# gregbugaj/marie-icr

Hardware: AMD Instinct MI355X
Metric: pages/sec (2550x3300, ~40 lines/page) (higher is better)
Workload: dtype f16; 1 GPU; BASELINE configs[2]: full detect->crop->recognize, 64 synthetic 2550x3300x3 u8 pages per GPU per step resident in HBM; DiT-base Mask R-CNN detector (resize to 1035x800, 1 pass, 8 pages per forward) + TrOCR-base recognizer on the generator's 40 ground-truth line boxes per page (fixed work), beam 3, 15+1 decoder steps; seeded random weights; f16 operands with fp32 accumulation is the 16-bit mode of ; crops_per_page=40

## Files before the change

include/marie_hip.h:

```cpp
#ifndef MARIE_HIP_H
#define MARIE_HIP_H

#include <stddef.h>
#include <stdint.h>

#ifdef __cplusplus
extern "C" {
#endif

#define MHIP_OK 0
#define MHIP_EINVAL (-22)
#define MHIP_ENOMEM (-12)
#define MHIP_EHIP (-5)
#define MHIP_ESTATE (-1)

#define MHIP_PREC_F16 0
#define MHIP_PREC_F32 1

typedef struct mhip_ctx mhip_ctx;
typedef struct mhip_crnn mhip_crnn;

int mhip_init(int device_id, mhip_ctx** out);
int mhip_destroy(mhip_ctx* ctx);
const char* mhip_last_error(mhip_ctx* ctx);
int mhip_set_stream(mhip_ctx* ctx, void* hip_stream);
int mhip_synchronize(mhip_ctx* ctx);
int mhip_device_info(mhip_ctx* ctx, char* arch, size_t arch_len, int* cu_count, size_t* hbm_bytes);
int mhip_memcpy_dev(mhip_ctx* ctx, void* dst_dev, const void* src_dev, size_t bytes);

typedef struct mhip_gate mhip_gate;
int mhip_gate_create(mhip_ctx* ctx, mhip_gate** out);
int mhip_gate_destroy(mhip_gate* g);
int mhip_gate_signal(mhip_gate* g, mhip_ctx* ctx);
long long mhip_gate_count(mhip_gate* g);
int mhip_gate_open(mhip_gate* g, int open);
int mhip_gate_wait(mhip_gate* g, mhip_ctx* ctx, long long seq, int timeout_ms);

int mhip_profile_enable(mhip_ctx* ctx, int enable);
int mhip_profile_reset(mhip_ctx* ctx);
int mhip_profile_read(mhip_ctx* ctx, int kernel_id, double* total_ms, int64_t* launches);
int mhip_profile_flops(mhip_ctx* ctx, int kernel_id, double* flops);
int mhip_kernel_count(void);
const char* mhip_kernel_name(int kernel_id);

typedef struct mhip_conv_desc {
  int32_t B, H, W, Cin;
  int32_t KH, KW, pad;
  int32_t N;
  int32_t pool, relu, out_f32;
  int32_t dil;
  int32_t Cin1;
  int32_t ldc;
  int32_t pad_cols_writable;
} mhip_conv_desc;
int mhip_conv2d_nhwc(mhip_ctx* ctx, int precision, const mhip_conv_desc* d, const void* in_dev,
                     const void* in2_dev, const void* w_dev, const float* scale_dev, const float* bias_dev,
                     void* out_dev);

typedef struct mhip_crop_desc {
  uint64_t src_offset;
  int32_t h, w, row_stride, channels;
} mhip_crop_desc;
int mhip_crop_batch(mhip_ctx* ctx, const uint8_t* base_dev, const mhip_crop_desc* descs_host, int n, int img_w,
                    uint8_t* out_dev);

int mhip_crnn_create(mhip_ctx* ctx, int precision, int num_class, mhip_crnn** out);
int mhip_crnn_destroy(mhip_crnn* m);

int mhip_crnn_set_tensor(mhip_crnn* m, const char* key, const float* data_host, const int64_t* shape, int ndim);
int mhip_crnn_finalize(mhip_crnn* m);
int mhip_crnn_alloc_arena(mhip_crnn* m);
int mhip_crnn_arena(mhip_crnn* m, void** arena_dev, size_t* bytes);

int mhip_crnn_seq_len(int w);

int mhip_crnn_forward(mhip_crnn* m, const uint8_t* crops_dev, int n, int w, float* logits_dev,
                      int32_t* argmax_dev, int32_t* tokens_dev, int32_t* lengths_dev, float* conf_dev);
int mhip_crnn_forward_host(mhip_crnn* m, const uint8_t* crops_host, int n, int w, float* logits_host,
                           int32_t* argmax_host, int32_t* tokens_host, int32_t* lengths_host,
                           float* conf_host);
int mhip_crnn_forward_crops(mhip_crnn* m, const uint8_t* base_dev, const mhip_crop_desc* descs_host, int n, int img_w,
                            float* logits_host, int32_t* argmax_host, int32_t* tokens_host, int32_t* lengths_host,
                            float* conf_host);
int mhip_crnn_forward_fragments_host(mhip_crnn* m, const uint8_t* packed_host, size_t packed_bytes,
                                     const mhip_crop_desc* descs_host, int n, int img_w, float* logits_host,
                                     int32_t* argmax_host, int32_t* tokens_host, int32_t* lengths_host,
                                     float* conf_host);
size_t mhip_crnn_workspace_bytes(mhip_crnn* m, int n, int w);
double mhip_crnn_kernel_flops(mhip_crnn* m, int kernel_id, int n, int w);

// ... 301 lines not shown
```

marie_icr_amd/_lib.py:

```python
from __future__ import annotations

import ctypes as C
import os
import weakref

import numpy as np

_HERE = os.path.dirname(os.path.abspath(__file__))
LIB_PATH = os.environ.get("MARIE_HIP_LIB") or os.path.join(_HERE, "libmarie_hip.so")

PREC_F16 = 0
PREC_F32 = 1

_vp, _i, _sz = C.c_void_p, C.c_int, C.c_size_t
_SIGNATURES = (
    ("mhip_init", _i, [_i, C.POINTER(_vp)]),
    ("mhip_destroy", _i, [_vp]),
    ("mhip_last_error", C.c_char_p, [_vp]),
    ("mhip_set_stream", _i, [_vp, _vp]),
    ("mhip_synchronize", _i, [_vp]),
    ("mhip_device_info", _i, [_vp, C.c_char_p, _sz, C.POINTER(_i), C.POINTER(_sz)]),
    ("mhip_memcpy_dev", _i, [_vp, _vp, _vp, _sz]),
    ("mhip_gate_create", _i, [_vp, C.POINTER(_vp)]),
    ("mhip_gate_destroy", _i, [_vp]),
    ("mhip_gate_signal", _i, [_vp, _vp]),
    ("mhip_gate_count", C.c_longlong, [_vp]),
    ("mhip_gate_open", _i, [_vp, _i]),
    ("mhip_gate_wait", _i, [_vp, _vp, C.c_longlong, _i]),
    ("mhip_profile_enable", _i, [_vp, _i]),
    ("mhip_profile_reset", _i, [_vp]),
    ("mhip_profile_read", _i, [_vp, _i, C.POINTER(C.c_double), C.POINTER(C.c_int64)]),
    ("mhip_profile_flops", _i, [_vp, _i, C.POINTER(C.c_double)]),
    ("mhip_kernel_count", _i, []),
    ("mhip_kernel_name", C.c_char_p, [_i]),
    ("mhip_conv2d_nhwc", _i, [_vp, _i, _vp, _vp, _vp, _vp, _vp, _vp, _vp]),
    ("mhip_icr_create", _i, [_vp, _i, _i, C.POINTER(_vp)]),
    ("mhip_icr_destroy", _i, [_vp]),
    ("mhip_icr_set_tensor", _i, [_vp, C.c_char_p, _vp, C.POINTER(C.c_int64), _i]),
    ("mhip_icr_finalize", _i, [_vp]),
    ("mhip_icr_alloc_arena", _i, [_vp]),
    ("mhip_icr_arena", _i, [_vp, C.POINTER(_vp), C.POINTER(_sz)]),
    ("mhip_icr_steps", _i, []),
    ("mhip_icr_forward", _i, [_vp, _vp, _i, _vp, _vp, _vp, _vp]),
    ("mhip_icr_forward_host", _i, [_vp, _vp, _i, _vp, _vp, _vp, _vp]),
    ("mhip_craft_create", _i, [_vp, _i, C.POINTER(_vp)]),
    ("mhip_craft_destroy", _i, [_vp]),
    ("mhip_craft_set_tensor", _i, [_vp, C.c_char_p, _vp, C.POINTER(C.c_int64), _i]),
    ("mhip_craft_finalize", _i, [_vp]),
    ("mhip_craft_alloc_arena", _i, [_vp]),
    ("mhip_craft_arena", _i, [_vp, C.POINTER(_vp), C.POINTER(_sz)]),
    ("mhip_craft_geometry", _i, [_i, _i, _i, C.c_double, C.POINTER(C.c_double), C.POINTER(_i), C.POINTER(_i),
                                 C.POINTER(_i), C.POINTER(_i)]),
    ("mhip_craft_workspace_bytes", _sz, [_vp, _i, _i, _i, C.c_double]),
    ("mhip_craft_kernel_flops", C.c_double, [_vp, _i, _i, _i, _i, C.c_double]),
    ("mhip_craft_forward", _i, [_vp, _vp, _i, _i, _i, C.c_double, _vp]),
    ("mhip_craft_detect", _i, [_vp, _vp, _i, _i, _i, C.c_double, C.c_float, C.c_float, C.c_float, _vp, _i,
                               C.POINTER(_i), _vp, C.POINTER(C.c_double)]),
    ("mhip_craft_detect_host", _i, [_vp, _vp, _i, _i, _i, C.c_double, C.c_float, C.c_float, C.c_float, _vp, _i,
                                    C.POINTER(_i), _vp, C.POINTER(C.c_double)]),
    ("mhip_craft_boxes_host", _i, [_vp, _vp, _i, _i, C.c_float, C.c_float, C.c_float, _vp, _i, C.POINTER(_i), _vp, _vp,
                                   _vp, _i, C.POINTER(_i)]),
    ("mhip_crop_batch", _i, [_vp, _vp, _vp, _i, _i, _vp]),
    ("mhip_pil_resize_rgb_host", _i, [_vp, _vp, _i, _i, _vp, _i, _i, _i]),
    ("mhip_vit_create", _i, [_vp, _i, _vp, C.POINTER(_vp)]),
    ("mhip_vit_destroy", _i, [_vp]),
    ("mhip_vit_set_tensor", _i, [_vp, C.c_char_p, _vp, C.POINTER(C.c_int64), _i]),
    ("mhip_vit_finalize", _i, [_vp]),
    ("mhip_vit_alloc_arena", _i, [_vp]),
# ... 80 lines not shown
    ("mhip_vq_kmeans_step_host", _i, [_vp, _vp, _i, _i, _vp, _vp, _i, _vp, _vp, _vp, C.POINTER(C.c_double)]),
    ("mhip_vq_heatmap_host", _i, [_vp, _vp, _i, _i, _i, _vp, _vp, _vp, _vp]),
    ("mhip_vq_peaks_host", _i, [_vp, _vp, _i, _i, _i, _vp, _i, _vp]),
    ("mhip_clip_cosine_host", _i, [_vp, _vp, _vp, _i, _i, _i, _vp]),
    ("mhip_max_page_size", _i, [_i, _i, _i, _i, C.c_double, C.POINTER(_i), C.POINTER(_i)]),
    ("mhip_resize_area_u8", _i, [_vp, _vp, _i, _i, _i, C.c_size_t, _vp, _i, _i]),
    ("mhip_resize_area_u8_host", _i, [_vp, _vp, _i, _i, _i, _vp, _i, _i]),
    ("mhip_resize_cubic_u8", _i, [_vp, _vp, _i, _i, _i, C.c_size_t, _vp, _i, _i]),
    ("mhip_resize_cubic_u8_host", _i, [_vp, _vp, _i, _i, _i, _vp, _i, _i]),
    ("mhip_merge_boxes", _i, [_vp, _i, _vp, C.POINTER(_i)]),
    ("mhip_line_merge", _i, [_vp, _i, _vp, C.POINTER(_i)]),
    ("mhip_find_line_numbers", _i, [_vp, _i, _vp, _i, _vp]),
    ("mhip_lines_from_bboxes", _i, [_vp, _i, _i, _i, _vp, _i, C.POINTER(_i)]),
    ("mhip_crnn_forward_crops", _i, [_vp, _vp, _vp, _i, _i, _vp, _vp, _vp, _vp, _vp]),
    ("mhip_crnn_forward_fragments_host", _i, [_vp, _vp, _sz, _vp, _i, _i, _vp, _vp, _vp, _vp, _vp]),
    ("mhip_crnn_create", _i, [_vp, _i, _i, C.POINTER(_vp)]),
    ("mhip_crnn_destroy", _i, [_vp]),
    ("mhip_crnn_set_tensor", _i, [_vp, C.c_char_p, _vp, C.POINTER(C.c_int64), _i]),
    ("mhip_crnn_finalize", _i, [_vp]),
    ("mhip_crnn_alloc_arena", _i, [_vp]),
    ("mhip_crnn_arena", _i, [_vp, C.POINTER(_vp), C.POINTER(_sz)]),
    ("mhip_crnn_seq_len", _i, [_i]),
    ("mhip_crnn_forward", _i, [_vp, _vp, _i, _i, _vp, _vp, _vp, _vp, _vp]),
    ("mhip_crnn_forward_host", _i, [_vp, _vp, _i, _i, _vp, _vp, _vp, _vp, _vp]),
    ("mhip_crnn_workspace_bytes", _sz, [_vp, _i, _i]),
    ("mhip_crnn_kernel_flops", C.c_double, [_vp, _i, _i, _i]),
)
EXPORTED_SYMBOLS = tuple(s[0] for s in _SIGNATURES)



class ConvDesc(C.Structure):
    _fields_ = [(n, C.c_int32) for n in ("B", "H", "W", "Cin", "KH", "KW", "pad", "N", "pool", "relu", "out_f32",
                                         "dil", "Cin1", "ldc", "pad_cols_writable")]


EPI_LN_ROWS, EPI_LN_COLS, EPI_SPLIT = 1, 2, 3


class GemmFoldDesc(C.Structure):
    _fields_ = ([(n, C.c_void_p) for n in ("in_dev", "w_dev", "scale_dev", "bias_dev", "out_dev", "ln_a_dev", "ln_b_dev",
                                           "ln_cs_dev", "row_bias_dev", "out2_dev", "res_dev", "res2_dev", "stats_dev")] +
                [(n, C.c_int32) for n in ("epi", "M", "N", "K", "act", "stats_ld", "row_period", "row_stride", "row_offset")])


class VitConfig(C.Structure):
    _fields_ = [("dim", C.c_int), ("depth", C.c_int), ("heads", C.c_int), ("patch", C.c_int), ("pos_h", C.c_int),
                ("pos_w", C.c_int), ("layer_scale", C.c_int), ("qkv_bias", C.c_int), ("final_norm", C.c_int),
                ("fpn", C.c_int), ("taps", C.c_int * 4), ("ln_eps", C.c_float)]


class DitConfig(C.Structure):
    _fields_ = [("model", C.c_int), ("min_size_test", C.c_int), ("max_size_test", C.c_int),
                ("detections_per_image", C.c_int), ("anchor_sizes", C.c_float * 5), ("aspect_ratios", C.c_float * 3),
                ("rpn_nms_thresh", C.c_float), ("score_thresh", C.c_float), ("nms_thresh", C.c_float),
                ("num_classes", C.c_int)]


class RegisterDesc(C.Structure):
    _fields_ = [("crop_x", C.c_int), ("crop_y", C.c_int), ("crop_w", C.c_int), ("crop_h", C.c_int), ("out_w", C.c_int),
                ("out_h", C.c_int), ("left", C.c_int), ("top", C.c_int), ("canvas_w", C.c_int), ("canvas_h", C.c_int),
                ("n_markers", C.c_int), ("marker_x", C.c_int * 4), ("marker_y", C.c_int * 4), ("marker_radius", C.c_int),
                ("marker_color", C.c_int * 3), ("final_w", C.c_int), ("final_h", C.c_int)]


class TrocrConfig(C.Structure):
    _fields_ = [("enc_dim", C.c_int), ("enc_depth", C.c_int), ("enc_heads", C.c_int), ("dec_dim", C.c_int),
# ... 67 lines not shown
            raise MarieHipError(f"mhip_init(device={device_id}) failed ({rc}): no usable HIP device")
        self.h = h
        self.lib = lib
        self.device_id = int(device_id)
        self._children = weakref.WeakSet()

    def adopt(self, child):
        self._children.add(child)

    def set_stream(self, stream_handle: int | None):
        check(self.h, self.lib.mhip_set_stream(self.h, C.c_void_p(stream_handle or 0)), "mhip_set_stream")

    def synchronize(self):
        check(self.h, self.lib.mhip_synchronize(self.h), "mhip_synchronize")

    def device_info(self):
        arch = C.create_string_buffer(64)
        cu = C.c_int()
        hbm = C.c_size_t()
        check(self.h, self.lib.mhip_device_info(self.h, arch, 64, C.byref(cu), C.byref(hbm)), "mhip_device_info")
        return {"arch": arch.value.decode(), "cu_count": cu.value, "hbm_bytes": hbm.value}

    def memcpy_dev(self, dst_ptr: int, src_ptr: int, nbytes: int):
        check(self.h, self.lib.mhip_memcpy_dev(self.h, C.c_void_p(dst_ptr), C.c_void_p(src_ptr), int(nbytes)),
              "mhip_memcpy_dev")

    def conv2d_nhwc(self, precision: int, desc: "ConvDesc", in_ptr: int, w_ptr: int, scale_ptr: int, bias_ptr: int,
                    out_ptr: int, in2_ptr: int = 0):
        check(self.h, self.lib.mhip_conv2d_nhwc(self.h, int(precision), C.byref(desc), C.c_void_p(in_ptr),
                                                C.c_void_p(in2_ptr or 0), C.c_void_p(w_ptr), C.c_void_p(scale_ptr or 0),
                                                C.c_void_p(bias_ptr or 0), C.c_void_p(out_ptr)),
              "mhip_conv2d_nhwc")

    def gemm_ln_fold(self, precision: int, desc: "GemmFoldDesc"):
        check(self.h, self.lib.mhip_gemm_ln_fold(self.h, int(precision), C.byref(desc)), "mhip_gemm_ln_fold")

    def ln_finalize(self, stats_ptr: int, chunks: int, ld: int, rstd_ptr: int, mur_ptr: int, rows: int, D: int, eps: float):
        check(self.h, self.lib.mhip_ln_finalize(self.h, C.c_void_p(stats_ptr), int(chunks), int(ld), C.c_void_p(rstd_ptr),
                                                C.c_void_p(mur_ptr), int(rows), int(D), float(eps)), "mhip_ln_finalize")

    def token_init_split(self, hi_ptr: int, lo_ptr: int, cls_row_ptr: int, cls_stats_ptr: int, stats_ptr: int, stats_ld: int,
                         B: int, npad: int, n_tok: int, D: int):
        check(self.h, self.lib.mhip_token_init_split(self.h, C.c_void_p(hi_ptr), C.c_void_p(lo_ptr), C.c_void_p(cls_row_ptr),
                                                     C.c_void_p(cls_stats_ptr), C.c_void_p(stats_ptr), int(stats_ld), int(B),
                                                     int(npad), int(n_tok), int(D)), "mhip_token_init_split")

    def profile_enable(self, on: bool):
        check(self.h, self.lib.mhip_profile_enable(self.h, 1 if on else 0), "mhip_profile_enable")

    def profile_reset(self):
        check(self.h, self.lib.mhip_profile_reset(self.h), "mhip_profile_reset")

    def profile_read(self):
        out = {}
        for k in range(self.lib.mhip_kernel_count()):
            ms = C.c_double()
            n = C.c_int64()
            check(self.h, self.lib.mhip_profile_read(self.h, k, C.byref(ms), C.byref(n)), "mhip_profile_read")
            fl = C.c_double()
            check(self.h, self.lib.mhip_profile_flops(self.h, k, C.byref(fl)), "mhip_profile_flops")
            out[self.lib.mhip_kernel_name(k).decode()] = {"id": k, "total_ms": ms.value, "launches": n.value,
                                                          "flops": fl.value}
        return out

    def make_gate(self) -> "PhaseGate":
        return PhaseGate(self)
# ... 102 lines not shown
```

marie_icr_amd/csrc/common.h:

```cpp
#pragma once
#include <hip/hip_runtime.h>
#include <stdint.h>
#include <stdio.h>
#include <string.h>

#include <mutex>
#include <string>
#include <vector>

#include "../../include/marie_hip.h"

enum MhipKernelId {
  MHIP_K_CONV_FIRST = 0,
  MHIP_K_CONV_IGEMM = 1,
  MHIP_K_LSTM_REC = 2,
  MHIP_K_CTC_DECODE = 3,
  MHIP_K_IMAGE_OPS = 4,
  MHIP_K_CCL = 5,
  MHIP_K_CROP_BATCH = 6,
  MHIP_K_ATTN = 7,
  MHIP_K_ATTN_FLASH = 8,
  MHIP_K_VIT_OPS = 9,
  MHIP_K_DET_OPS = 10,
  MHIP_K_DEC_OPS = 11,
  MHIP_K_IGEMM_T64 = 12,
  MHIP_K_IGEMM_T128 = 13,
  MHIP_K_IGEMM_T256 = 14,
  MHIP_K_IGEMM_S128 = 15,
  MHIP_K_IGEMM_PATCH = 16,
  MHIP_K_CROSS_ATTN = 17,
  MHIP_K_ATTN_BIAS = 18,
  MHIP_K_VQ_ASSIGN = 19,
  MHIP_K_VQ_KMEANS = 20,
  MHIP_K_VQ_HEATMAP = 21,
  MHIP_K_VQ_PEAKS = 22,
  MHIP_K_CLIP_COSINE = 23,
  MHIP_K_COUNT = 24
};

constexpr int MHIP_ZERO_BYTES = 65536;

struct ProfSlot {
  double total_ms = 0.0;
  int64_t launches = 0;
  double flops = 0.0;
  int parent = -1;
  std::vector<std::pair<hipEvent_t, hipEvent_t>> pending;
};

struct mhip_ctx {
  int device = 0;
  hipStream_t stream = nullptr;
  std::string err;
  void* ws = nullptr;
  size_t ws_bytes = 0;
  void* zeros = nullptr;
  bool profiling = false;
  ProfSlot prof[MHIP_K_COUNT];
  std::vector<hipEvent_t> event_pool;
  struct PinnedRing {
    static constexpr int N = 4;
    void* buf[N] = {nullptr, nullptr, nullptr, nullptr};
    size_t cap[N] = {0, 0, 0, 0};
    hipEvent_t ev[N] = {nullptr, nullptr, nullptr, nullptr};
    int next = 0;
  } stage;
};
int mhip_stage_h2d(mhip_ctx* ctx, void* dst_dev, const void* src_host, size_t bytes);

int mhip_fail(mhip_ctx* ctx, int code, const char* fmt, ...);
inline void mhip_quiesce(const mhip_ctx* ctx) {
  if (ctx) (void)hipSetDevice(ctx->device);
  (void)hipDeviceSynchronize();
}
int mhip_ensure_workspace(mhip_ctx* ctx, size_t bytes);

struct Carver {
  char* base;
  size_t align;
  size_t off = 0;
  explicit Carver(void* b, size_t a = 256) : base((char*)b), align(a) {}
  template <typename P = char>
  P* take(size_t bytes) {
    const size_t at = off;
    off = (off + bytes + align - 1) / align * align;
    return base ? (P*)(base + at) : nullptr;
  }
  Carver sub(size_t a) const { return Carver(base ? base + off : nullptr, a); }
};

template <typename F>
size_t mhip_layout_bytes(F&& layout, size_t align = 256) {
  Carver c(nullptr, align);
  layout(c);
  return c.off;
}
template <typename F>
int mhip_carve_workspace(mhip_ctx* ctx, F&& layout, size_t align = 256) {
  const size_t need = mhip_layout_bytes(layout, align);
  int rc = mhip_ensure_workspace(ctx, need);
  if (rc) return rc;
  Carver ws(ctx->ws, align);
  layout(ws);
// ... 334 lines not shown
```

marie_icr_amd/csrc/context.hip:

```cpp
#include <stdarg.h>

#include <algorithm>

#include "common.h"

int mhip_fail(mhip_ctx* ctx, int code, const char* fmt, ...) {
  char buf[512];
  va_list ap;
  va_start(ap, fmt);
  vsnprintf(buf, sizeof(buf), fmt, ap);
  va_end(ap);
  if (ctx) ctx->err = buf;
  return code;
}

static const char* kKernelNames[MHIP_K_COUNT] = {"conv_first", "conv_igemm", "lstm_rec",   "ctc_decode",
                                                 "image_ops",  "ccl",        "crop_batch", "attn",
                                                 "attn_flash", "vit_ops",    "det_ops",    "dec_ops",
                                                 "conv_igemm<64>", "conv_igemm<128>", "conv_igemm<256>", "conv_igemm<1128>",
                                                 "conv3x3_patch", "cross_attn", "attn_bias",
                                                 "vq_assign", "vq_kmeans", "vq_heatmap", "vq_peaks", "clip_cosine"};

extern "C" int mhip_kernel_count(void) { return MHIP_K_COUNT; }
extern "C" const char* mhip_kernel_name(int k) { return (k >= 0 && k < MHIP_K_COUNT) ? kKernelNames[k] : ""; }

extern "C" int mhip_init(int device_id, mhip_ctx** out) {
  if (!out) return MHIP_EINVAL;
  *out = nullptr;
  int ndev = 0;
  if (hipGetDeviceCount(&ndev) != hipSuccess || ndev <= 0) return MHIP_EHIP;
  if (device_id < 0 || device_id >= ndev) return MHIP_EINVAL;
  if (hipSetDevice(device_id) != hipSuccess) return MHIP_EHIP;
  mhip_ctx* ctx = new mhip_ctx();
  ctx->device = device_id;
  for (int k = MHIP_K_IGEMM_T64; k <= MHIP_K_IGEMM_PATCH; ++k) ctx->prof[k].parent = MHIP_K_CONV_IGEMM;
  if (hipMalloc(&ctx->zeros, MHIP_ZERO_BYTES) != hipSuccess || hipMemset(ctx->zeros, 0, MHIP_ZERO_BYTES) != hipSuccess) {
    delete ctx;
// ... 38 lines not shown
    r.cap[i] = cap;
  }
  memcpy(r.buf[i], src_host, bytes);
  MHIP_HIP(ctx, hipMemcpyAsync(dst_dev, r.buf[i], bytes, hipMemcpyHostToDevice, ctx->stream));
  MHIP_HIP(ctx, hipEventRecord(r.ev[i], ctx->stream));
  return MHIP_OK;
}

extern "C" const char* mhip_last_error(mhip_ctx* ctx) { return ctx ? ctx->err.c_str() : "null ctx"; }

extern "C" int mhip_set_stream(mhip_ctx* ctx, void* s) {
  if (!ctx) return MHIP_EINVAL;
  ctx->stream = (hipStream_t)s;
  return MHIP_OK;
}

extern "C" int mhip_synchronize(mhip_ctx* ctx) {
  if (!ctx) return MHIP_EINVAL;
  MHIP_HIP(ctx, hipStreamSynchronize(ctx->stream));
  return MHIP_OK;
}

extern "C" int mhip_device_info(mhip_ctx* ctx, char* arch, size_t arch_len, int* cu_count, size_t* hbm_bytes) {
  if (!ctx) return MHIP_EINVAL;
  hipDeviceProp_t p;
  MHIP_HIP(ctx, hipGetDeviceProperties(&p, ctx->device));
  if (arch && arch_len) {
    strncpy(arch, p.gcnArchName, arch_len - 1);
    arch[arch_len - 1] = 0;
  }
  if (cu_count) *cu_count = p.multiProcessorCount;
  if (hbm_bytes) *hbm_bytes = p.totalGlobalMem;
  return MHIP_OK;
}

extern "C" int mhip_memcpy_dev(mhip_ctx* ctx, void* dst, const void* src, size_t bytes) {
  if (!ctx || (bytes && (!dst || !src))) return MHIP_EINVAL;
  MHIP_HIP(ctx, hipMemcpyAsync(dst, src, bytes, hipMemcpyDeviceToDevice, ctx->stream));
  return MHIP_OK;
}

int mhip_ensure_workspace(mhip_ctx* ctx, size_t bytes) {
  if (bytes <= ctx->ws_bytes) return MHIP_OK;
  MHIP_HIP(ctx, hipStreamSynchronize(ctx->stream));
  if (ctx->ws) MHIP_HIP(ctx, hipFree(ctx->ws));
  ctx->ws = nullptr;
  ctx->ws_bytes = 0;
  size_t want = bytes + bytes / 8;
  if (hipMalloc(&ctx->ws, want) != hipSuccess) {
    (void)hipGetLastError();
    return mhip_fail(ctx, MHIP_ENOMEM, "workspace allocation of %zu bytes failed", want);
  }
  ctx->ws_bytes = want;
  return MHIP_OK;
}

static hipEvent_t get_event(mhip_ctx* ctx) {
  if (!ctx->event_pool.empty()) {
    hipEvent_t e = ctx->event_pool.back();
    ctx->event_pool.pop_back();
    return e;
  }
  hipEvent_t e = nullptr;
  (void)hipEventCreate(&e);
  return e;
}
// ... 58 lines not shown
```

marie_icr_amd/csrc/conv_igemm.hip:

```cpp
#include <stdlib.h>

#include <type_traits>

#include "igemm_common.h"

using namespace igemm;

namespace {

template <int BN_>
struct Cfg {
  static constexpr bool SMALL = BN_ / 1000 == 1;
  static constexpr int BN = BN_ % 1000;
  static constexpr int BM = SMALL ? 128 : ((BN == 64) ? 512 : 256);
  static constexpr int WN = BN / 64;
  static constexpr int WM = 8 / WN;
  static constexpr int MT = BM / WM / 16;
  static constexpr int NSTAGE = SMALL ? 4 : ((BN == 128) ? 3 : 2);
  static constexpr int A_BYTES = BM * ROWB;
  static constexpr int B_BYTES = BN * ROWB;
  static constexpr int STAGE_BYTES = A_BYTES + B_BYTES;
  static constexpr int RPI = 64 * 16 / ROWB;
  static constexpr int ACHUNKS = BM * (ROWB / 16) / NTHREADS;
  static constexpr int WCHUNKS = BN * (ROWB / 16) / NTHREADS;
  static constexpr int GL = ACHUNKS + WCHUNKS;
  static constexpr int EPW = BN < 128 ? BN : 128;
  static constexpr int EPI_BYTES = BM * (EPW * 4 + 16);
  static constexpr int RING_BYTES = NSTAGE * STAGE_BYTES;
  static constexpr int LDS_BYTES = RING_BYTES > EPI_BYTES ? RING_BYTES : EPI_BYTES;
};

__device__ __forceinline__ float gelu_erf(float t) {
  const float x = t * 0.70710678118654752f, ax = fabsf(x);
  const float u = __builtin_amdgcn_rcpf(__builtin_fmaf(0.3275911f, ax, 1.f));
  float poly = __builtin_fmaf(1.061405429f, u, -1.453152027f);
  poly = __builtin_fmaf(poly, u, 1.421413741f);
  poly = __builtin_fmaf(poly, u, -0.284496736f);
// ... 787 lines not shown
      return mhip_fail(ctx, MHIP_EINVAL, "conv_igemm: a concatenated input needs a 1x1, unpadded, unpooled conv");
    if (d.Cin1 <= 0 || d.Cin1 >= d.Cin || d.Cin1 % bke != 0)
      return mhip_fail(ctx, MHIP_EINVAL, "conv_igemm: Cin1=%d must split Cin=%d on a multiple of %d", d.Cin1, d.Cin, bke);
  }
  if (a.Ho <= 0 || a.Wo <= 0) return mhip_fail(ctx, MHIP_EINVAL, "conv_igemm: empty output %dx%d", a.Ho, a.Wo);
  a.Hp = a.Ho; a.Wp = a.Wo;
  long long M;
  if (d.pool == POOL_2x2) {
    a.Hp = a.Ho / 2; a.Wp = a.Wo / 2;
    M = (long long)d.B * a.Hp * a.Wp * 4;
  } else if (d.pool == POOL_2x1) {
    a.Hp = a.Ho / 2;
    M = (long long)d.B * a.Hp * a.Wo * 2;
  } else {
    M = (long long)d.B * a.Ho * a.Wo;
  }
  if (M <= 0 || M > 0x7fffffffLL - 512) return mhip_fail(ctx, MHIP_EINVAL, "conv_igemm: M=%lld out of range", M);
  a.M = (int)M;
  a.N = d.N;
  a.Ktot = d.KH * d.KW * d.Cin;
  a.cpt = d.Cin / bke;
  a.nslices = d.KH * d.KW * a.cpt;
  a.relu = d.relu;
  a.out_f32 = d.out_f32;
  a.PH = a.PW = a.tiles_x = a.tiles_y = 0;
  const double fl = ctx->profiling ? mhip_conv_flops(d) : 0.0;
  if (ctx->profiling) ctx->prof[MHIP_K_CONV_IGEMM].flops += fl;
  if (d.epi == EPI_NONE) {
    const int r = mhip_try_launch_conv3x3_patch(ctx, precision, d, a);
    if (r == 0) ctx->prof[MHIP_K_IGEMM_PATCH].flops += fl;
    if (r <= 0) return r;
  }
  static const int force_bn = getenv("MARIE_HIP_FORCE_BN") ? atoi(getenv("MARIE_HIP_FORCE_BN")) : 0;
  const int bn = force_bn ? force_bn : ((a.N > 128) ? 256 : ((a.N > 64 || d.epi != EPI_NONE) ? 128 : 64));
  const int bm = (bn == 64) ? 512 : 256;
  a.mtiles = (a.M + bm - 1) / bm;
  a.ntiles = (a.N + bn - 1) / bn;
  static const bool mid_off = getenv("MARIE_HIP_NO_MID_TILE") != nullptr;
  int tile = bn == 256 ? 256 : (bn == 128 ? 128 : 64);
  if (!mid_off && bn == 256 && a.mtiles * a.ntiles < 192 && a.mtiles * ((a.N + 127) / 128) >= 192 && !force_bn) {
    a.ntiles = (a.N + 127) / 128;
    ctx->prof[MHIP_K_IGEMM_T128].flops += fl;
    tile = 128;
  } else if (a.mtiles * a.ntiles < 192 && (a.N > 64 || d.epi != EPI_NONE) && d.pool == POOL_NONE && !d.in2) {
    a.mtiles = (a.M + 127) / 128;
    a.ntiles = (a.N + 127) / 128;
    ctx->prof[MHIP_K_IGEMM_S128].flops += fl;
    tile = 1128;
  } else {
    ctx->prof[bn == 64 ? MHIP_K_IGEMM_T64 : (bn == 128 ? MHIP_K_IGEMM_T128 : MHIP_K_IGEMM_T256)].flops += fl;
  }
  return precision == MHIP_PREC_F16 ? launch_tile<_Float16>(ctx, a, d.pool, tile) : launch_tile<float>(ctx, a, d.pool, tile);
}
```

marie_icr_amd/csrc/crnn_api.hip:

```cpp
#include <math.h>

#include <memory>

#include "weights_util.h"

extern "C" int mhip_conv2d_nhwc(mhip_ctx* ctx, int precision, const mhip_conv_desc* d, const void* in,
                                const void* in2, const void* w, const float* scale, const float* bias, void* out) {
  if (!ctx || !d) return MHIP_EINVAL;
  if (precision != MHIP_PREC_F16 && precision != MHIP_PREC_F32)
    return mhip_fail(ctx, MHIP_EINVAL, "unknown precision %d", precision);
  if (d->B < 1 || d->H < 1 || d->W < 1 || d->N < 1 || d->KH < 1 || d->KW < 1 || d->pad < 0 || d->pool < 0 ||
      d->pool > 2)
    return mhip_fail(ctx, MHIP_EINVAL, "conv2d: bad descriptor");
  MHIP_HIP(ctx, hipSetDevice(ctx->device));
  ConvDesc c;
  c.in = in; c.w = w; c.scale = scale; c.bias = bias; c.out = out;
  c.B = d->B; c.H = d->H; c.W = d->W; c.Cin = d->Cin;
  c.KH = d->KH; c.KW = d->KW; c.pad = d->pad;
  c.N = d->N; c.pool = d->pool; c.relu = d->relu; c.out_f32 = d->out_f32;
  c.dil = d->dil > 0 ? d->dil : 1;
  c.in2 = in2; c.Cin1 = d->Cin1;
  c.ldc = d->ldc; c.pad_cols_writable = d->pad_cols_writable;
  return mhip_launch_conv_igemm(ctx, precision, c);
}

namespace {

struct ConvSpec {
  const char* key;
  int co, ci, kh, kw;
  bool has_bias;
  const char* bn;
};
const ConvSpec kConvs[7] = {
    {"FeatureExtraction.ConvNet.0", 64, 1, 3, 3, true, nullptr},
    {"FeatureExtraction.ConvNet.3", 128, 64, 3, 3, true, nullptr},
    {"FeatureExtraction.ConvNet.6", 256, 128, 3, 3, true, nullptr},
    {"FeatureExtraction.ConvNet.8", 256, 256, 3, 3, true, nullptr},
    {"FeatureExtraction.ConvNet.11", 512, 256, 3, 3, false, "FeatureExtraction.ConvNet.12"},
    {"FeatureExtraction.ConvNet.14", 512, 512, 3, 3, false, "FeatureExtraction.ConvNet.15"},
    {"FeatureExtraction.ConvNet.18", 512, 512, 2, 2, true, nullptr},
};

struct Layout {
  size_t conv0_w = 0, conv0_b = 0;
  size_t conv_w[7] = {0}, conv_scale[7] = {0}, conv_bias[7] = {0};
  size_t ih_w[2] = {0}, ih_b[2] = {0}, hh_pack[2] = {0}, lin_w[2] = {0}, lin_b[2] = {0};
  size_t pred_w = 0, pred_b = 0;
};

}

struct mhip_crnn {
  mhip_ctx* ctx = nullptr;
  int precision = MHIP_PREC_F16;
// ... 382 lines not shown
```

marie_icr_amd/csrc/phase_gate.hip:

```cpp
#include <chrono>
#include <condition_variable>

#include "common.h"

struct mhip_gate {
  static constexpr int RING = 16;
  int device = 0;
  std::mutex mu;
  std::condition_variable cv;
  long long count = 0;
  bool open = false;
  hipEvent_t ev[RING] = {};
};

extern "C" int mhip_gate_create(mhip_ctx* ctx, mhip_gate** out) {
  if (!ctx || !out) return MHIP_EINVAL;
  *out = nullptr;
  MHIP_HIP(ctx, hipSetDevice(ctx->device));
  mhip_gate* g = new mhip_gate();
  g->device = ctx->device;
  for (int i = 0; i < mhip_gate::RING; ++i) {
    hipError_t e = hipEventCreateWithFlags(&g->ev[i], hipEventDisableTiming);
    if (e != hipSuccess) {
      for (int j = 0; j < i; ++j) (void)hipEventDestroy(g->ev[j]);
      delete g;
      return mhip_fail(ctx, MHIP_EHIP, "gate: hipEventCreate: %s", hipGetErrorString(e));
    }
  }
  *out = g;
  return MHIP_OK;
}

extern "C" int mhip_gate_destroy(mhip_gate* g) {
  if (!g) return MHIP_OK;
  {
    std::lock_guard<std::mutex> lk(g->mu);
    g->open = true;
  }
  g->cv.notify_all();
  (void)hipSetDevice(g->device);
  for (auto e : g->ev) (void)hipEventDestroy(e);
  delete g;
  return MHIP_OK;
}

extern "C" int mhip_gate_signal(mhip_gate* g, mhip_ctx* ctx) {
  if (!g || !ctx) return MHIP_EINVAL;
  if (ctx->device != g->device) return mhip_fail(ctx, MHIP_EINVAL, "gate: context on device %d, gate on %d", ctx->device, g->device);
  {
    std::lock_guard<std::mutex> lk(g->mu);
    MHIP_HIP(ctx, hipEventRecord(g->ev[(g->count + 1) % mhip_gate::RING], ctx->stream));
    ++g->count;
  }
  g->cv.notify_all();
  return MHIP_OK;
}

extern "C" long long mhip_gate_count(mhip_gate* g) {
  if (!g) return MHIP_EINVAL;
  std::lock_guard<std::mutex> lk(g->mu);
  return g->count;
}

extern "C" int mhip_gate_open(mhip_gate* g, int open) {
  if (!g) return MHIP_EINVAL;
  {
    std::lock_guard<std::mutex> lk(g->mu);
    g->open = open != 0;
  }
  g->cv.notify_all();
  return MHIP_OK;
}

extern "C" int mhip_gate_wait(mhip_gate* g, mhip_ctx* ctx, long long seq, int timeout_ms) {
  if (!g || !ctx || seq < 1) return MHIP_EINVAL;
  if (ctx->device != g->device) return mhip_fail(ctx, MHIP_EINVAL, "gate: context on device %d, gate on %d", ctx->device, g->device);
  std::unique_lock<std::mutex> lk(g->mu);
  const bool ok = g->cv.wait_for(lk, std::chrono::milliseconds(timeout_ms < 0 ? 0 : timeout_ms), [&] { return g->open || g->count >= seq; });
  if (!ok || g->open) return 0;
  MHIP_HIP(ctx, hipSetDevice(ctx->device));
  MHIP_HIP(ctx, hipStreamWaitEvent(ctx->stream, g->ev[g->count % mhip_gate::RING], 0));
  return 1;
}
```

Before: 96.94 pages/s.

## Add cost-model tile planner splitting igemm rows into big-tile and tail segments

Replaces the fixed threshold-based tile selection in the implicit-GEMM conv launcher with a planner that models per-tile cost and wave quantization from the actual CU count. For pure 1x1 GEMMs it can split M into two launches, a full-wave big-tile segment and a smaller-tile tail, to reduce last-wave idle CUs. Multi-launch splitting is disabled when the context shares the device via phase gates. The change also adds a residual pointer to the conv descriptor and exposes the planner through the API. It costs extra launches and relies on hardcoded timing constants.

```diff
diff --git a/include/marie_hip.h b/include/marie_hip.h
--- a/include/marie_hip.h
+++ b/include/marie_hip.h
@@ -52,10 +52,32 @@
   int32_t Cin1;
   int32_t ldc;
   int32_t pad_cols_writable;
+  const void* res_dev;
 } mhip_conv_desc;
 int mhip_conv2d_nhwc(mhip_ctx* ctx, int precision, const mhip_conv_desc* d, const void* in_dev,
                      const void* in2_dev, const void* w_dev, const float* scale_dev, const float* bias_dev,
                      void* out_dev);
+
+#define MHIP_IGEMM_EPI_PLAIN 0
+#define MHIP_IGEMM_EPI_GELU 1
+#define MHIP_IGEMM_EPI_RES32 2
+#define MHIP_IGEMM_EPI_SPLIT 3
+typedef struct mhip_igemm_constraints {
+  int32_t epilogue;
+  int32_t folded;
+  int32_t one_shape;
+  int32_t no_small_tile;
+  int32_t row_period;
+  int32_t force_tile;
+  int32_t no_mid_tile;
+  int32_t elem_bytes;
+} mhip_igemm_constraints;
+typedef struct mhip_igemm_segment {
+  int32_t first_row, rows, tile;
+} mhip_igemm_segment;
+int mhip_igemm_plan(int M, int N, int K, const mhip_igemm_constraints* c, int n_cu, mhip_igemm_segment* segs, int max_segs,
+                    double* modelled_us);
+int mhip_set_plan_cu_count(mhip_ctx* ctx, int n_cu);
 
 typedef struct mhip_crop_desc {
   uint64_t src_offset;
diff --git a/marie_icr_amd/_lib.py b/marie_icr_amd/_lib.py
--- a/marie_icr_amd/_lib.py
+++ b/marie_icr_amd/_lib.py
@@ -34,6 +34,8 @@
     ("mhip_kernel_count", _i, []),
     ("mhip_kernel_name", C.c_char_p, [_i]),
     ("mhip_conv2d_nhwc", _i, [_vp, _i, _vp, _vp, _vp, _vp, _vp, _vp, _vp]),
+    ("mhip_igemm_plan", _i, [_i, _i, _i, _vp, _i, _vp, _i, C.POINTER(C.c_double)]),
+    ("mhip_set_plan_cu_count", _i, [_vp, _i]),
     ("mhip_icr_create", _i, [_vp, _i, _i, C.POINTER(_vp)]),
     ("mhip_icr_destroy", _i, [_vp]),
     ("mhip_icr_set_tensor", _i, [_vp, C.c_char_p, _vp, C.POINTER(C.c_int64), _i]),
@@ -180,7 +182,29 @@
 
 class ConvDesc(C.Structure):
     _fields_ = [(n, C.c_int32) for n in ("B", "H", "W", "Cin", "KH", "KW", "pad", "N", "pool", "relu", "out_f32",
-                                         "dil", "Cin1", "ldc", "pad_cols_writable")]
+                                         "dil", "Cin1", "ldc", "pad_cols_writable")] + [("res_dev", C.c_void_p)]
+
+
+IGEMM_EPI_PLAIN, IGEMM_EPI_GELU, IGEMM_EPI_RES32, IGEMM_EPI_SPLIT = 0, 1, 2, 3
+
+
+class IgemmConstraints(C.Structure):
+    _fields_ = [(n, C.c_int32) for n in ("epilogue", "folded", "one_shape", "no_small_tile", "row_period", "force_tile",
+                                         "no_mid_tile", "elem_bytes")]
+
+
+class IgemmSegment(C.Structure):
+    _fields_ = [(n, C.c_int32) for n in ("first_row", "rows", "tile")]
+
+
+def igemm_plan(M: int, N: int, K: int, n_cu: int, **constraints):
+    c = IgemmConstraints(**{"elem_bytes": 2, **constraints})
+    segs = (IgemmSegment * 4)()
+    us = C.c_double()
+    n = load().mhip_igemm_plan(int(M), int(N), int(K), C.byref(c), int(n_cu), segs, 4, C.byref(us))
+    if n < 1:
+        raise MarieHipError(f"mhip_igemm_plan({M}, {N}, {K}, n_cu={n_cu}) failed ({n})")
+    return [(segs[i].first_row, segs[i].rows, segs[i].tile) for i in range(n)], us.value
 
 
 EPI_LN_ROWS, EPI_LN_COLS, EPI_SPLIT = 1, 2, 3
@@ -314,6 +338,9 @@
                                                 C.c_void_p(bias_ptr or 0), C.c_void_p(out_ptr)),
               "mhip_conv2d_nhwc")
 
+    def set_plan_cu_count(self, n_cu: int):
+        check(self.h, self.lib.mhip_set_plan_cu_count(self.h, int(n_cu)), "mhip_set_plan_cu_count")
+
     def gemm_ln_fold(self, precision: int, desc: "GemmFoldDesc"):
         check(self.h, self.lib.mhip_gemm_ln_fold(self.h, int(precision), C.byref(desc)), "mhip_gemm_ln_fold")
 
diff --git a/marie_icr_amd/csrc/common.h b/marie_icr_amd/csrc/common.h
--- a/marie_icr_amd/csrc/common.h
+++ b/marie_icr_amd/csrc/common.h
@@ -56,6 +56,10 @@
   size_t ws_bytes = 0;
   void* zeros = nullptr;
   bool profiling = false;
+  int device_cu = 0;
+  int plan_cu = 0;
+  int shares_device = 0;
+  int plan_force_tile = 0;
   ProfSlot prof[MHIP_K_COUNT];
   std::vector<hipEvent_t> event_pool;
   struct PinnedRing {
@@ -69,6 +73,7 @@
 int mhip_stage_h2d(mhip_ctx* ctx, void* dst_dev, const void* src_host, size_t bytes);
 
 int mhip_fail(mhip_ctx* ctx, int code, const char* fmt, ...);
+int mhip_plan_cu_count(mhip_ctx* ctx);
 inline void mhip_quiesce(const mhip_ctx* ctx) {
   if (ctx) (void)hipSetDevice(ctx->device);
   (void)hipDeviceSynchronize();
diff --git a/marie_icr_amd/csrc/context.hip b/marie_icr_amd/csrc/context.hip
--- a/marie_icr_amd/csrc/context.hip
+++ b/marie_icr_amd/csrc/context.hip
@@ -3,6 +3,7 @@
 #include <algorithm>
 
 #include "common.h"
+#include "igemm_plan.h"
 
 int mhip_fail(mhip_ctx* ctx, int code, const char* fmt, ...) {
   char buf[512];
@@ -107,6 +108,37 @@
   if (cu_count) *cu_count = p.multiProcessorCount;
   if (hbm_bytes) *hbm_bytes = p.totalGlobalMem;
   return MHIP_OK;
+}
+
+int mhip_plan_cu_count(mhip_ctx* ctx) {
+  if (ctx->plan_cu > 0) return ctx->plan_cu;
+  if (ctx->device_cu <= 0) {
+    int n = 0;
+    MHIP_HIP(ctx, hipDeviceGetAttribute(&n, hipDeviceAttributeMultiprocessorCount, ctx->device));
+    if (n <= 0) return mhip_fail(ctx, MHIP_EHIP, "device %d reports %d compute units", ctx->device, n);
+    ctx->device_cu = n;
+  }
+  return ctx->device_cu;
+}
+
+extern "C" int mhip_set_plan_cu_count(mhip_ctx* ctx, int n_cu) {
+  if (!ctx) return MHIP_EINVAL;
+  ctx->plan_cu = n_cu > 0 ? n_cu : 0;
+  return MHIP_OK;
+}
+
+extern "C" int mhip_igemm_plan(int M, int N, int K, const mhip_igemm_constraints* c, int n_cu, mhip_igemm_segment* segs, int max_segs,
+                               double* modelled_us) {
+  if (!c || !segs || max_segs < 1) return MHIP_EINVAL;
+  igplan::Constraints pc;
+  pc.kind = c->epilogue; pc.folded = c->folded; pc.one_shape = c->one_shape; pc.no_small = c->no_small_tile;
+  pc.row_period = c->row_period; pc.force_tile = c->force_tile; pc.no_mid = c->no_mid_tile;
+  pc.elem_bytes = c->elem_bytes == 4 ? 4 : 2;
+  const igplan::Plan p = igplan::igemm_plan(M, N, K, pc, n_cu);
+  if (p.n < 1 || p.n > max_segs) return MHIP_EINVAL;
+  for (int s = 0; s < p.n; ++s) { segs[s].first_row = p.seg[s].first_row; segs[s].rows = p.seg[s].rows; segs[s].tile = p.seg[s].tile; }
+  if (modelled_us) *modelled_us = p.us;
+  return p.n;
 }
 
 extern "C" int mhip_memcpy_dev(mhip_ctx* ctx, void* dst, const void* src, size_t bytes) {
diff --git a/marie_icr_amd/csrc/conv_igemm.hip b/marie_icr_amd/csrc/conv_igemm.hip
--- a/marie_icr_amd/csrc/conv_igemm.hip
+++ b/marie_icr_amd/csrc/conv_igemm.hip
@@ -3,6 +3,7 @@
 #include <type_traits>
 
 #include "igemm_common.h"
+#include "igemm_plan.h"
 
 using namespace igemm;
 
@@ -856,23 +857,50 @@
     if (r <= 0) return r;
   }
   static const int force_bn = getenv("MARIE_HIP_FORCE_BN") ? atoi(getenv("MARIE_HIP_FORCE_BN")) : 0;
-  const int bn = force_bn ? force_bn : ((a.N > 128) ? 256 : ((a.N > 64 || d.epi != EPI_NONE) ? 128 : 64));
-  const int bm = (bn == 64) ? 512 : 256;
-  a.mtiles = (a.M + bm - 1) / bm;
-  a.ntiles = (a.N + bn - 1) / bn;
   static const bool mid_off = getenv("MARIE_HIP_NO_MID_TILE") != nullptr;
-  int tile = bn == 256 ? 256 : (bn == 128 ? 128 : 64);
-  if (!mid_off && bn == 256 && a.mtiles * a.ntiles < 192 && a.mtiles * ((a.N + 127) / 128) >= 192 && !force_bn) {
-    a.ntiles = (a.N + 127) / 128;
-    ctx->prof[MHIP_K_IGEMM_T128].flops += fl;
-    tile = 128;
-  } else if (a.mtiles * a.ntiles < 192 && (a.N > 64 || d.epi != EPI_NONE) && d.pool == POOL_NONE && !d.in2) {
-    a.mtiles = (a.M + 127) / 128;
-    a.ntiles = (a.N + 127) / 128;
-    ctx->prof[MHIP_K_IGEMM_S128].flops += fl;
-    tile = 1128;
-  } else {
-    ctx->prof[bn == 64 ? MHIP_K_IGEMM_T64 : (bn == 128 ? MHIP_K_IGEMM_T128 : MHIP_K_IGEMM_T256)].flops += fl;
-  }
-  return precision == MHIP_PREC_F16 ? launch_tile<_Float16>(ctx, a, d.pool, tile) : launch_tile<float>(ctx, a, d.pool, tile);
-}
+  const bool gemm = d.KH == 1 && d.KW == 1 && d.pad == 0 && a.pad_x == 0 && a.sy == 1 && d.pool == POOL_NONE && !d.in2;
+  igplan::Constraints pc;
+  pc.kind = d.epi == EPI_SPLIT ? igplan::KIND_SPLIT
+            : (d.relu == ACT_GELU ? igplan::KIND_GELU : ((d.out_f32 && d.res) ? igplan::KIND_RES32 : igplan::KIND_PLAIN));
+  pc.folded = d.epi != EPI_NONE;
+  pc.one_shape = !gemm || d.epi == EPI_LN_COLS || ctx->shares_device;
+  pc.no_small = d.pool != POOL_NONE || d.in2 != nullptr;
+  pc.row_period = d.row_period;
+  pc.force_tile = force_bn ? force_bn : ctx->plan_force_tile;
+  pc.no_mid = mid_off;
+  pc.elem_bytes = esz;
+  int rc = mhip_plan_cu_count(ctx);
+  if (rc < 0) return rc;
+  const igplan::Plan plan = igplan::igemm_plan(a.M, a.N, a.Ktot, pc, rc);
+  if (plan.n < 1) return mhip_fail(ctx, MHIP_EINVAL, "conv_igemm: no legal tile shape for M=%d N=%d (forced tile %d)", a.M, a.N, pc.force_tile);
+  const int oe = d.out_f32 ? 4 : esz;
+  const size_t grow = (size_t)(a.ldc ? a.ldc : a.N) * oe;
+  const IgemmArgs whole = a;
+  for (int s = 0; s < plan.n; ++s) {
+    const igplan::Segment& sg = plan.seg[s];
+    a = whole;
+    if (plan.n > 1) {
+      const size_t r0 = (size_t)sg.first_row;
+      a.in = whole.in + r0 * (size_t)d.Cin * esz;
+      a.B = 1; a.H = a.Ho = a.Hp = 1; a.W = a.Wo = a.Wp = sg.rows;
+      a.M = sg.rows;
+      if (d.row_period) {
+        a.row_offset = whole.row_offset + (int)(r0 / d.row_period) * d.row_stride;
+      } else {
+        a.out = whole.out + r0 * grow;
+        if (whole.res) a.res = whole.res + r0 * grow;
+        if (whole.out2) a.out2 = whole.out2 + r0 * grow;
+        if (whole.res2) a.res2 = whole.res2 + r0 * grow;
+        if (whole.stats) a.stats = whole.stats + r0 * 2;
+      }
+      if (d.epi == EPI_LN_ROWS) { a.ln_a = whole.ln_a + r0; a.ln_b = whole.ln_b + r0; }
+    }
+    a.mtiles = (a.M + igplan::tile_rows(sg.tile) - 1) / igplan::tile_rows(sg.tile);
+    a.ntiles = (a.N + igplan::tile_cols(sg.tile) - 1) / igplan::tile_cols(sg.tile);
+    const int slot = sg.tile == 1128 ? MHIP_K_IGEMM_S128 : (sg.tile == 64 ? MHIP_K_IGEMM_T64 : (sg.tile == 128 ? MHIP_K_IGEMM_T128 : MHIP_K_IGEMM_T256));
+    ctx->prof[slot].flops += fl * ((double)sg.rows / (double)whole.M);
+    rc = precision == MHIP_PREC_F16 ? launch_tile<_Float16>(ctx, a, d.pool, sg.tile) : launch_tile<float>(ctx, a, d.pool, sg.tile);
+    if (rc) return rc;
+  }
+  return 0;
+}
diff --git a/marie_icr_amd/csrc/crnn_api.hip b/marie_icr_amd/csrc/crnn_api.hip
--- a/marie_icr_amd/csrc/crnn_api.hip
+++ b/marie_icr_amd/csrc/crnn_api.hip
@@ -21,6 +21,7 @@
   c.dil = d->dil > 0 ? d->dil : 1;
   c.in2 = in2; c.Cin1 = d->Cin1;
   c.ldc = d->ldc; c.pad_cols_writable = d->pad_cols_writable;
+  c.res = d->res_dev;
   return mhip_launch_conv_igemm(ctx, precision, c);
 }
 
diff --git a/marie_icr_amd/csrc/igemm_plan.h b/marie_icr_amd/csrc/igemm_plan.h
--- /dev/null
+++ b/marie_icr_amd/csrc/igemm_plan.h
@@ -0,0 +1,131 @@
+#pragma once
+#include <stdint.h>
+
+#include <initializer_list>
+
+namespace igplan {
+
+enum { TILE_64 = 64, TILE_128 = 128, TILE_256 = 256, TILE_S128 = 1128 };
+enum { KIND_PLAIN = 0, KIND_GELU = 1, KIND_RES32 = 2, KIND_SPLIT = 3, KIND_COUNT = 4 };
+
+struct Constraints {
+  int kind = KIND_PLAIN;
+  int folded = 0;
+  int one_shape = 0;
+  int no_small = 0;
+  int row_period = 0;
+  int force_tile = 0;
+  int no_mid = 0;
+  int elem_bytes = 2;
+};
+
+struct Segment { int first_row, rows, tile; };
+struct Plan {
+  int n = 0;
+  Segment seg[2];
+  double us = 0.0;
+};
+
+inline int tile_rows(int tile) { return tile == TILE_S128 ? 128 : (tile == TILE_64 ? 512 : 256); }
+inline int tile_cols(int tile) { return tile == TILE_S128 ? 128 : tile; }
+
+constexpr double T_SLICE[4] =      {0.97,   0.97,    1.67,    0.61};
+constexpr double T_FIXED[KIND_COUNT][4] = {
+             {4.5,    4.5,     7.2,     1.6},
+             {6.7,    6.7,     10.6,    2.9},
+             {12.8,   12.8,    24.1,    5.8},
+             {12.0,   12.0,    22.5,    5.6}};
+constexpr double T_LAUNCH = 0.0;
+constexpr double F32_SLICE_FACTOR = 8.0;
+
+inline int shape_index(int tile) { return tile == TILE_64 ? 0 : (tile == TILE_128 ? 1 : (tile == TILE_256 ? 2 : 3)); }
+
+inline double tile_us(int tile, int kind, int slices, int elem_bytes) {
+  const int s = shape_index(tile);
+  return T_FIXED[kind][s] + slices * T_SLICE[s] * (elem_bytes == 4 ? F32_SLICE_FACTOR : 1.0);
+}
+
+inline long long tiles_of(long long rows, int N, int tile) {
+  return ((rows + tile_rows(tile) - 1) / tile_rows(tile)) * ((N + tile_cols(tile) - 1) / tile_cols(tile));
+}
+
+inline bool legal(int tile, int N, const Constraints& c) {
+  const bool narrow = N <= 64 && !c.folded;
+  switch (tile) {
+    case TILE_64: return narrow;
+    case TILE_128: return !narrow && !(c.no_mid && N > 128);
+    case TILE_256: return !narrow && N > 128;
+    case TILE_S128: return !narrow && !c.no_small;
+    default: return false;
+  }
+}
+
+inline double segment_us(long long rows, int N, int slices, int tile, const Constraints& c, int n_cu) {
+  const long long t = tiles_of(rows, N, tile);
+  return (double)((t + n_cu - 1) / n_cu) * tile_us(tile, c.kind, slices, c.elem_bytes);
+}
+
+inline int threshold_tile(int M, int N, const Constraints& c, int n_cu) {
+  if (legal(TILE_64, N, c)) return TILE_64;
+  const long long enough = 3LL * n_cu / 4, mt = (M + 255) / 256;
+  if (N > 128) {
+    if (mt * ((N + 255) / 256) >= enough) return TILE_256;
+    if (!c.no_mid && mt * ((N + 127) / 128) >= enough) return TILE_128;
+    return c.no_small ? TILE_256 : TILE_S128;
+  }
+  return (mt >= enough || c.no_small) ? TILE_128 : TILE_S128;
+}
+
+inline Plan single(int M, int N, int slices, int tile, const Constraints& c, int n_cu) {
+  Plan p;
+  p.n = 1;
+  p.seg[0] = {0, M, tile};
+  p.us = segment_us(M, N, slices, tile, c, n_cu);
+  return p;
+}
+
+inline Plan igemm_plan(int M, int N, int K, const Constraints& c, int n_cu) {
+  Plan best;
+  if (M <= 0 || N <= 0 || K <= 0 || n_cu <= 0 || c.kind < 0 || c.kind >= KIND_COUNT) return best;
+  const int slices = (int)(((long long)K * c.elem_bytes + 127) / 128);
+  if (c.force_tile) {
+    const int t = c.force_tile;
+    if ((t != TILE_64 && t != TILE_128 && t != TILE_256 && t != TILE_S128) || (t == TILE_S128 && c.no_small) ||
+        (t == TILE_64 && c.folded))
+      return best;
+    return single(M, N, slices, t, c, n_cu);
+  }
+  const int base = threshold_tile(M, N, c, n_cu);
+  const long long bt = tiles_of(M, N, base), last = bt - (bt - 1) / n_cu * n_cu;
+  if (c.one_shape || 4 * last >= 3LL * n_cu) return single(M, N, slices, base, c, n_cu);
+  auto offer = [&](const Plan& p) { if (!best.n || p.us < best.us) best = p; };
+  offer(single(M, N, slices, base, c, n_cu));
+  for (int tile : {TILE_256, TILE_128, TILE_S128})
+    if (tile != base && legal(tile, N, c)) offer(single(M, N, slices, tile, c, n_cu));
+  for (int big : {TILE_256, TILE_128}) {
+    if (!legal(big, N, c)) continue;
+    const long long ntn = (N + tile_cols(big) - 1) / tile_cols(big), mtiles = (M + 255) / 256;
+    const long long R = mtiles * ntn / n_cu;
+    if (R < 1) continue;
+    long long rows1 = (R * n_cu / ntn) * 256;
+    if (c.row_period > 0) {
+      long long a = 256, b = c.row_period;
+      while (b) { const long long t = a % b; a = b; b = t; }
+      const long long lcm = 256 / a * c.row_period;
+      rows1 = rows1 / lcm * lcm;
+    }
+    if (rows1 <= 0 || rows1 >= M) continue;
+    for (int rest : {TILE_128, TILE_S128}) {
+      if (rest == big || !legal(rest, N, c)) continue;
+      Plan p;
+      p.n = 2;
+      p.seg[0] = {0, (int)rows1, big};
+      p.seg[1] = {(int)rows1, (int)(M - rows1), rest};
+      p.us = segment_us(rows1, N, slices, big, c, n_cu) + segment_us(M - rows1, N, slices, rest, c, n_cu) + T_LAUNCH;
+      offer(p);
+    }
+  }
+  return best;
+}
+
+}
diff --git a/marie_icr_amd/csrc/phase_gate.hip b/marie_icr_amd/csrc/phase_gate.hip
--- a/marie_icr_amd/csrc/phase_gate.hip
+++ b/marie_icr_amd/csrc/phase_gate.hip
@@ -10,6 +10,7 @@
   std::condition_variable cv;
   long long count = 0;
   bool open = false;
+  bool waited = false;
   hipEvent_t ev[RING] = {};
 };
 
@@ -51,6 +52,7 @@
     std::lock_guard<std::mutex> lk(g->mu);
     MHIP_HIP(ctx, hipEventRecord(g->ev[(g->count + 1) % mhip_gate::RING], ctx->stream));
     ++g->count;
+    if (g->waited) ctx->shares_device = 1;
   }
   g->cv.notify_all();
   return MHIP_OK;
@@ -80,5 +82,7 @@
   if (!ok || g->open) return 0;
   MHIP_HIP(ctx, hipSetDevice(ctx->device));
   MHIP_HIP(ctx, hipStreamWaitEvent(ctx->stream, g->ev[g->count % mhip_gate::RING], 0));
+  g->waited = true;
+  ctx->shares_device = 1;
   return 1;
 }
```

New measurement: 96.93 pages/s, median of 2. No clear change (-0.0%).
